# clinfo/kGCN

Hardware: AMD Instinct MI355X
Metric: graphs/sec GraphConv fwd+bwd, 32-node mol graphs x64 feat (higher is better)
Workload: dtype f32

## Files before the change

include/kgcn_hip.h:

```cpp
#ifndef KGCN_HIP_H_
#define KGCN_HIP_H_

#include <stdint.h>

#ifdef __cplusplus
extern "C" {
#endif

#define KGCN_HIP_ABI_VERSION 2

#define KGCN_PAD_COL 32

#define KGCN_ROW_PAD_COMPACT 0x104
#define KGCN_CSR_UNIT_VALUES 1


typedef struct kgcn_csr_batch {
  int32_t num_graphs;
  int32_t rows;
  int32_t cols;
  int32_t max_nnz_per_graph;
  int32_t row_pad;
  int32_t reserved_;
  int64_t nnz;
// ... 123 lines not shown
int kgcn_dense_fwd_act_f32(const float* x, int64_t m, int32_t din, int64_t x_ld, const float* w, int64_t w_ld,
                           int32_t trans_w, const float* bias, float* y, int32_t dout, int64_t y_ld, int32_t act,
                           void* stream);
int64_t kgcn_dense_fwd_workspace_bytes(int32_t din, int32_t dout);
int kgcn_dense_fwd_ws_f32(const float* x, int64_t m, int32_t din, int64_t x_ld, const float* w, int64_t w_ld,
                          int32_t trans_w, const float* bias, float* y, int32_t dout, int64_t y_ld, int32_t act,
                          void* workspace, int64_t workspace_bytes, void* stream);
#define KGCN_WTABLE_MAX_JOBS 16
typedef struct kgcn_wtable_job {
  const float* w;
  int64_t w_ld;
  int32_t trans_w, k, n;
  int32_t k_w;
  void* table;
  const float* extra_row;
} kgcn_wtable_job;
int kgcn_wtable_split_multi(const kgcn_wtable_job* jobs, int32_t num_jobs, void* stream);
int kgcn_dense_fwd_tab_f32(const float* x, int64_t m, int32_t din, int64_t x_ld, const float* w, int64_t w_ld,
                           int32_t trans_w, const float* bias, float* y, int32_t dout, int64_t y_ld, int32_t act,
                           const void* table, int64_t table_bytes, void* stream);
int kgcn_dense_dx_dact_f32(const float* grad, const float* act_out, int64_t m, int32_t dout, int64_t ld, const float* w,
                           int64_t w_ld, int32_t din, float* dx, int64_t dx_ld, int32_t act, float* dpre,
                           void* workspace, int64_t workspace_bytes, void* stream);
int kgcn_dense_dx_dact_tab_f32(const float* grad, const float* act_out, int64_t m, int32_t dout, int64_t ld, const float* w,
                               int64_t w_ld, int32_t din, float* dx, int64_t dx_ld, int32_t act, float* dpre, const void* table,
                               int64_t table_bytes, void* stream);
int kgcn_dense_dx_dact_gather_supported(int64_t m, int32_t din, int32_t dout);
int kgcn_dense_dx_dact_gather_f32(const float* grad, const float* pooled_grad, int64_t pooled_ld, int32_t n_nodes,
                                  const float* act_out, int64_t m, int32_t dout, int64_t ld, const float* w, int64_t w_ld,
                                  int32_t din, float* dx, int64_t dx_ld, int32_t act, float* dpre, void* table,
                                  int64_t table_bytes, int32_t table_ready, void* stream);
int kgcn_dense_bwd_supported(int64_t m, int32_t din, int32_t dout);
int kgcn_dense_bwd_f32(const float* grad, const float* pooled_grad, int64_t pooled_ld, int32_t n_nodes, const float* act_out,
                       int32_t act, int64_t ld, const float* x, int64_t x_ld, int64_t m, int32_t din, int32_t dout,
                       const float* w, int64_t w_ld, float* dx, int64_t dx_ld, float* dw, float* dbias, void* table,
                       int64_t table_bytes, int32_t table_ready, void* workspace, int64_t workspace_bytes, void* stream);
int kgcn_dense_bwd_dot_f32(const float* grad, const float* act_out, int32_t act, int64_t ld, const float* x, int64_t x_ld, int64_t m,
                           int32_t din, int32_t dout, const float* w, int64_t w_ld, const float* dotx, int64_t dotx_ld, float* dw,
                           float* dbias, float* dot_out, void* table, int64_t table_bytes, int32_t table_ready, void* workspace,
                           int64_t workspace_bytes, void* stream);
int kgcn_dense_dx_dact_dot_supported(int64_t m, int32_t din, int32_t dout);
int64_t kgcn_dense_dx_dact_dot_workspace_bytes(int64_t m, int32_t din);
int kgcn_dense_dx_dact_dot_f32(const float* grad, const float* act_out, int64_t m, int32_t dout, int64_t ld, const float* w,
                               int64_t w_ld, int32_t din, const float* dotx, int64_t dotx_ld, int32_t act, float* dpre,
                               void* table, int64_t table_bytes, int32_t table_ready, float* dot_out, void* workspace,
                               int64_t workspace_bytes, void* stream);
int kgcn_act_fwd_f32(const float* x, int64_t n, int32_t act, float* y, void* stream);
int kgcn_act_bwd_f32(const float* act_out, const float* grad, int64_t n, int32_t act, float* dpre, void* stream);

int64_t kgcn_graph_bn_workspace_bytes(int32_t d);
int kgcn_graph_bn_stats_f32(const float* x, int64_t graphs, int32_t n_nodes, int32_t d, const int32_t* enabled,
                            float* mean, float* var, void* workspace, int64_t workspace_bytes, void* stream);
int kgcn_graph_bn_apply_f32(const float* x, int64_t graphs, int32_t n_nodes, int32_t d, const int32_t* enabled,
                            const float* mean, const float* var, const float* gamma, const float* beta, float eps,
                            float* y, void* stream);
int kgcn_graph_bn_bwd_f32(const float* x, const float* grad, int64_t graphs, int32_t n_nodes, int32_t d,
                          const int32_t* enabled, const float* mean, const float* var, const float* gamma, float eps,
                          int32_t training, float* dx, float* dgamma, float* dbeta, void* workspace,
                          int64_t workspace_bytes, void* stream);

int kgcn_graph_bn_apply_act_f32(const float* x, int64_t graphs, int32_t n_nodes, int32_t d, const int32_t* enabled,
                                const float* mean, const float* var, const float* gamma, const float* beta, float eps,
                                int32_t act, float* y, void* stream);
int kgcn_graph_bn_bwd_dact_f32(const float* x, const float* grad, const float* act_out, int32_t act, int64_t graphs,
                               int32_t n_nodes, int32_t d, const int32_t* enabled, const float* mean, const float* var,
                               const float* gamma, float eps, int32_t training, float* dx, float* dgamma, float* dbeta,
                               void* workspace, int64_t workspace_bytes, void* stream);

int64_t kgcn_coo_pack_workspace_bytes(int64_t nnz, int32_t num_graphs, int32_t rows, int32_t cols);
int kgcn_coo_pack_f32(const int32_t* graph, const int32_t* row, const int32_t* col, const float* val, int64_t nnz,
                      int32_t num_graphs, int32_t rows, int32_t cols, int32_t transposed, int32_t* rowptr_out,
                      void* cv_out, int32_t* perm_out, int32_t* stats_out, void* workspace, int64_t workspace_bytes,
                      void* stream);
int64_t kgcn_csr_pad4_workspace_bytes(int32_t num_graphs, int32_t rows);
int kgcn_csr_pad4(const kgcn_csr_batch* a, int32_t* rowptr4_out, void* cv4_out, int64_t cv4_capacity,
                  int32_t* slots_out, int32_t* graph_ptr_out, int32_t* stats_out, void* workspace,
                  int64_t workspace_bytes, void* stream);
int64_t kgcn_compact_values_offset(int64_t nnz);
int64_t kgcn_compact_cv_words(int64_t nnz, int32_t with_values);
int kgcn_csr_compact4(const kgcn_csr_batch* a4, void* cv_out, int with_values, void* slots_out, int32_t* stats_out,
                      void* stream);
int kgcn_graphconv_fused_reads_compact(int32_t backward, int32_t num_graphs, int32_t n_nodes, int32_t din, int32_t dout,
                                       int32_t max_nnz_per_graph, int32_t with_dx);

int64_t kgcn_ragged_workspace_bytes(int32_t num_sel);
int kgcn_ragged_plan(const kgcn_csr_batch* src, const int32_t* sizes, const int32_t* sel, int32_t num_sel,
                     int32_t* graph_ptr, int32_t* entry_ptr, void* workspace, int64_t workspace_bytes, void* stream);
int kgcn_ragged_compact_csr(const kgcn_csr_batch* src, const int32_t* sel, int32_t num_sel, const int32_t* graph_ptr,
                            const int32_t* entry_ptr, int32_t capacity_rows, int32_t* dst_rowptr, int32_t* dst_cv,
                            int64_t dst_cv_capacity, int32_t* status, void* stream);
int kgcn_ragged_compact_csr_pair(const kgcn_csr_batch* src, const kgcn_csr_batch* src_t, const int32_t* sel, int32_t num_sel,
                                 const int32_t* graph_ptr, const int32_t* entry_ptr, int32_t capacity_rows, int32_t* dst_rowptr,
                                 int32_t* dst_cv, int64_t dst_cv_capacity, int32_t* dst_t_rowptr, int32_t* dst_t_cv,
                                 int64_t dst_t_cv_capacity, int32_t* status, void* stream);
#define KGCN_RAGGED_BLOCK_ROWS 32
int32_t kgcn_ragged_block_rows(void);
int32_t kgcn_ragged_num_blocks(int32_t capacity_rows);
int kgcn_ragged_blocks(const int32_t* graph_ptr, int32_t num_sel, int32_t capacity_rows, int32_t* block_ptr, void* stream);
int kgcn_ragged_compact_rows_f32(const float* src, const int32_t* sel, int32_t num_sel, int32_t n_nodes, int32_t d,
                                 const int32_t* graph_ptr, int32_t capacity_rows, float* dst, void* stream);
int kgcn_ragged_compact_rows_aug_f32(const float* src, const int32_t* sel, int32_t num_sel, int32_t n_nodes, int32_t d,
                                     const int32_t* graph_ptr, int32_t capacity_rows, float* dst, int32_t dst_ld, void* stream);
int kgcn_ragged_expand_rows_f32(const float* src, int32_t num_graphs, int32_t n_nodes, int32_t d,
                                const int32_t* graph_ptr, int32_t fill_row, float* dst, void* stream);
int kgcn_ragged_gather_fwd_f32(const float* x, const int32_t* graph_ptr, int64_t batch, int32_t n_nodes, int32_t d,
                               int32_t pad_row, float* out, void* stream);
int64_t kgcn_ragged_gather_bwd_workspace_bytes(int32_t d);
int kgcn_ragged_gather_bwd_f32(const float* dout_grad, const int32_t* graph_ptr, int64_t batch, int32_t n_nodes, int32_t d,
                               int32_t pad_row, int32_t capacity_rows, float* dx, void* workspace, int64_t workspace_bytes,
                               void* stream);

int64_t kgcn_loss_workspace_bytes(int64_t batch);
int kgcn_masked_sigmoid_ce_f32(const float* logits, const float* labels, const float* mask, const float* mask_label,
                               int64_t batch, int32_t tasks, int32_t weighted, float pos_weight,
                               const float* pos_weight_per_task, float* cost, float* dlogits, float* sums, void* workspace,
                               int64_t workspace_bytes, void* stream);
int kgcn_masked_softmax_ce_f32(const float* logits, const float* labels, const float* mask, int64_t batch, int32_t classes,
                               float* cost, float* dlogits, float* sums, void* workspace, int64_t workspace_bytes,
                               void* stream);
int kgcn_sparse_softmax_ce_f32(const float* logits, const int64_t* label_idx, const float* mask, int64_t batch,
                               int32_t classes, float* cost, float* dlogits, float* sums, void* workspace,
                               int64_t workspace_bytes, void* stream);
int kgcn_loss_grad_f32(const float* dlogits, const float* g_opt, const float* g_sum, int64_t batch, int64_t n, float* out,
                       void* stream);
int kgcn_adam_tf_f32(float* params, const float* grads, float* m, float* v, int64_t n, float lr, float beta1, float beta2,
                     float eps, int64_t* step_counter, void* stream);
#define KGCN_ADAM_MAX_SEGMENTS 32
typedef struct kgcn_adam_segment {
  const float* grad;
  int64_t offset, numel;
} kgcn_adam_segment;
int kgcn_adam_tf_multi_f32(float* params, float* m, float* v, int64_t n, const kgcn_adam_segment* segments, int32_t num_segments,
                           float lr, float beta1, float beta2, float eps, int64_t* step_counter, void* stream);

int kgcn_augment_ones_f32(const float* x, int64_t m, int32_t din, int64_t x_ld, float* out, int64_t out_ld, void* stream);
int kgcn_augment_ones_bwd_f32(const float* dout_grad, int64_t m, int32_t din, int64_t g_ld, float* dx, int64_t dx_ld,
                              void* stream);

#define KGCN_STACK_MAX_LAYERS 8
typedef struct kgcn_stack_layer {
  int32_t kind, act, din, dout;
  const float* w;
  const float* b;
  const float* mean;
  const float* var;
  float eps;
  int32_t route;
} kgcn_stack_layer;
int kgcn_gcn_stack_supported(int32_t n_nodes, int32_t max_nnz_per_graph, const kgcn_stack_layer* layers, int32_t num_layers);
int64_t kgcn_gcn_stack_param_floats(const kgcn_stack_layer* layers, int32_t num_layers);
int kgcn_gcn_stack_fwd_f32(const kgcn_csr_batch* a, const float* x, const int32_t* enabled, const kgcn_stack_layer* layers,
                           int32_t num_layers, float* const* layer_out, float* pooled, void* stream);
int64_t kgcn_gcn_stack_bwd_workspace_bytes(int32_t num_graphs, const kgcn_stack_layer* layers, int32_t num_layers);
int kgcn_gcn_stack_bwd_f32(const kgcn_csr_batch* at, const float* x, const int32_t* enabled, const kgcn_stack_layer* layers,
                           int32_t num_layers, float* const* layer_out, const float* dlast, int32_t gather, float* dx,
                           float* dparams, void* workspace, int64_t workspace_bytes, void* stream);

int kgcn_reduce_defer(int32_t on);
int kgcn_reduce_pending(void);
int kgcn_reduce_flush(void* stream);

int kgcn_dense_mfma_products(int32_t kind, int64_t m, int32_t din, int32_t dout);

enum {
  KGCN_SPMM_NONE = 0,
  KGCN_SPMM_TILE = 1,
// ... 227 lines not shown
```

kgcn_amd/csrc/fused.hip:

```cpp
#include <type_traits>

#include "kgcn_common.h"
#include "kgcn_probe.h"

namespace kgcn {

constexpr int FN = 32;
constexpr int FD = 64;
constexpr int ALD = 68;
constexpr int BLD = 65;
constexpr int MAX_WPB = 8;


KP_BUFFER(g_probe, kgcn_probe_set)

__device__ __forceinline__ void wave_sync() {
  __builtin_amdgcn_wave_barrier();
  asm volatile("" ::: "memory");
  __builtin_amdgcn_wave_barrier();
}

typedef int i32x4 __attribute__((ext_vector_type(4)));

__device__ __forceinline__ f32x4 ldv4(const float* p) { return *reinterpret_cast<const f32x4*>(p); }
// ... 276 lines not shown
      x1 = ldv4(reinterpret_cast<const float*>(sb + (cw[0] >> 16)));
      x2 = ldv4(reinterpret_cast<const float*>(sb + (cw[1] & 0xffffu)));
      x3 = ldv4(reinterpret_cast<const float*>(sb + (cw[1] >> 16)));
    }
  }
  template <int I>
  __device__ __forceinline__ float val() const {
    if constexpr (LAY == LAY_PAD4) return __int_as_float(I == 0 ? q0.y : I == 1 ? q0.w : I == 2 ? q1.y : q1.w);
    else return v[I];
  }
  __device__ __forceinline__ void fma() {
    if constexpr (LAY == LAY_UNIT) {
      a = x0;
      add4(a, x1); add4(a, x2); add4(a, x3);
    } else {
      const float v0 = val<0>();
      a[0] = v0 * x0[0]; a[1] = v0 * x0[1]; a[2] = v0 * x0[2]; a[3] = v0 * x0[3];
      fma4(a, val<1>(), x1);
      fma4(a, val<2>(), x2);
      fma4(a, val<3>(), x3);
    }
  }
};
template <int LAY>
__device__ __forceinline__ f32x4 gather4(const int2* ecv, const float* ev, const float* srcl, int k) {
  Grp4<LAY> q;
  q.ecv(ecv, ev, k);
  q.tile(srcl);
  f32x4 a0 = {0.f, 0.f, 0.f, 0.f};
  if constexpr (LAY == LAY_UNIT) {
    add4(a0, q.x0); add4(a0, q.x1); add4(a0, q.x2); add4(a0, q.x3);
  } else {
    fma4(a0, q.template val<0>(), q.x0); fma4(a0, q.template val<1>(), q.x1);
    fma4(a0, q.template val<2>(), q.x2); fma4(a0, q.template val<3>(), q.x3);
  }
  return a0;
}
template <int LAY>
__device__ __forceinline__ void grp_tail(f32x4& a, int s, int len, const int2* ecv, const float* ev, const float* srcl) {
  if (__builtin_amdgcn_ballot_w64(len > 4)) {
    for (int k = 4; __builtin_amdgcn_ballot_w64(k < len); k += 4)
      if (k < len) add4(a, gather4<LAY>(ecv, ev, srcl, s + k));
  }
}

template <typename Emit>
__device__ __forceinline__ void aggregate_rows(const int2* ecv, const int* tab, const float* tile,
                                               int N, int dcols, int lane, Emit&& emit) {
  const int sub = lane >> 4, cl = lane & 15;
  const float* srcl = tile + cl * 4;
  const bool col_ok = cl * 4 < dcols;
  for (int j0 = 0; j0 < N; j0 += 4) {
    const int j = j0 + sub;
    const bool ok = (j < N) && col_ok;
    int s_, len, row;
    unpack_slot(tab[ok ? j : 0], s_, len, row);
    if (!ok) len = 0;
    f32x4 acc = {0.f, 0.f, 0.f, 0.f};
    for (int k = 0; __builtin_amdgcn_ballot_w64(k < len); k += 4)
      if (k < len) add4(acc, gather4<LAY_PAD4>(ecv, nullptr, srcl, s_ + k));
    if (ok) emit(row, cl, acc);
  }
}

template <int LAY, typename Emit>
__device__ __forceinline__ void aggregate_rows_full(const int2* ecv, const float* ev, const int* tab, const float* tile,
                                                    int lane, Emit&& emit) {
  const int sub = lane >> 4, cl = lane & 15;
  const float* srcl = tile + cl * 4;
#pragma unroll
  for (int p8 = 0; p8 < 8; ++p8) {
    int s, len, row;
    unpack_slot(tab[4 * p8 + sub], s, len, row);
    Grp4<LAY> q;
    q.ecv(ecv, ev, s);
    q.tile(srcl);
    q.fma();
    grp_tail<LAY>(q.a, s, len, ecv, ev, srcl);
    emit(row, cl, q.a);
    __builtin_amdgcn_sched_barrier(0);
  }
}

constexpr int A_FWD = FN * ALD;
constexpr int A_BWD = FN * BLD;

template <bool FULL>
__device__ __forceinline__ void load_w_frags(float (&wr0)[32], float (&wr1)[32],
                                             const float* __restrict__ w, int din, int dout, int li,
                                             int hi) {
#pragma unroll
  for (int s = 0; s < 32; ++s) {
    const int k = hi * 32 + s;
    if constexpr (FULL) {
      wr0[s] = w[k * FD + li];
      wr1[s] = w[k * FD + 32 + li];
    } else {
      wr0[s] = (k < din && li < dout) ? w[(long)k * dout + li] : 0.f;
      wr1[s] = (k < din && 32 + li < dout) ? w[(long)k * dout + 32 + li] : 0.f;
    }
  }
}

__device__ __forceinline__ void store_c_tiles(float* tile, const f32x16& c0, const f32x16& c1, int li,
                                              int hi) {
#pragma unroll
  for (int r = 0; r < 16; ++r) {
    const int row = (r & 3) + 8 * (r >> 2) + 4 * hi;
    tile[row * FD + li] = c0[r];
    tile[row * FD + 32 + li] = c1[r];
  }
}

template <int MODE>
__global__ __launch_bounds__(512, 2) void graphconv_fwd_kernel(
    const int* __restrict__ slots, const int* __restrict__ gptr, const int2* __restrict__ cv,
    const float* __restrict__ x, const float* __restrict__ w, const float* __restrict__ bias,
    float* __restrict__ out, int T, int N, int din, int dout, int max_nnz, int pack) {
  constexpr bool VEC = MODE == 2;
  extern __shared__ __attribute__((aligned(16))) unsigned char smem[];
  const int tid = threadIdx.x;
  const int wave = tid >> 6, lane = tid & 63;
  const int li = lane & 31, hi = lane >> 5;
  const int wpb = blockDim.x >> 6;
  WaveSlice ws = carve(smem, wave, max_nnz * pack, A_FWD, 1);

  const int stride = gridDim.x * wpb * pack;
  int t = __builtin_amdgcn_readfirstlane((blockIdx.x * wpb + wave) * pack);
  if (t >= T) return;

  for (int i = lane; i < A_FWD; i += 64) ws.a[i] = 0.f;
  for (int i = lane; i < FD; i += 64) ws.b[FN * FD + i] = 0.f;

  float wr0[32], wr1[32];
  load_w_frags<false>(wr0, wr1, w, din, dout, li, hi);
  const float b0 = (bias && li < dout) ? bias[li] : 0.f;
  const float b1 = (bias && 32 + li < dout) ? bias[32 + li] : 0.f;

  auto graphs_at = [&](int tt) { return T - tt < pack ? T - tt : pack; };
  int P = graphs_at(t);

  TileRegs fx;
  CsrRegs fc;
  MetaRegs m_cur, m_nxt;
  issue_meta_p(m_cur, slots, gptr, t, P, N, lane);
  int base = meta_base(m_cur), cnt = meta_cnt_p(m_cur, P);
  issue_tile_g<MODE>(fx, x + (long)t * N * din, P * N * din, lane);
  issue_cv(fc, cv, base, cnt, lane);
  int tn = t + stride;
  int Pn = graphs_at(tn < T ? tn : t);
  issue_meta_p(m_nxt, slots, gptr, tn < T ? tn : t, Pn, N, lane);
  wave_sync();

  for (;;) {
    const int rows = P * N;
    land_tile_g<MODE>(fx, ws.a, ALD, rows * din, din, lane);
    land_csr_p(fc, ws.ecv, ws.rp, cv, m_cur, base, cnt, N, P, lane);
    wave_sync();

    const bool has_next = tn < T;
    const int tp = has_next ? tn : t;
    const int base_n = meta_base(m_nxt), cnt_n = meta_cnt_p(m_nxt, Pn);
    issue_tile_g<MODE>(fx, x + (long)tp * N * din, Pn * N * din, lane);
    issue_cv(fc, cv, base_n, cnt_n, lane);
    m_cur = m_nxt;
    const int P_next = Pn;
    {
      const int tnn = tn + stride;
      const int tq = tnn < T ? tnn : tp;
      Pn = graphs_at(tq);
      issue_meta_p(m_nxt, slots, gptr, tq, Pn, N, lane);
    }

    f32x16 acc0, acc1;
#pragma unroll
    for (int r = 0; r < 16; ++r) { acc0[r] = b0; acc1[r] = b1; }
    {
      f32x4 a4[8];
#pragma unroll
      for (int q = 0; q < 8; ++q) a4[q] = ldv4(ws.a + li * ALD + hi * 32 + q * 4);
#pragma unroll
      for (int s = 0; s < 32; ++s) {
        const float a = a4[s >> 2][s & 3];
        acc0 = __builtin_amdgcn_mfma_f32_32x32x2f32(a, wr0[s], acc0, 0, 0, 0);
        acc1 = __builtin_amdgcn_mfma_f32_32x32x2f32(a, wr1[s], acc1, 0, 0, 0);
      }
    }
    store_c_tiles(ws.b, acc0, acc1, li, hi);
    wave_sync();

    float* ot = out + (long)t * N * dout;
    aggregate_rows(ws.ecv, ws.rp, ws.b, rows, dout, lane, [&](int r, int cl, f32x4 acc) {
      if constexpr (VEC) {
        stv4(ot + (long)r * dout + cl * 4, acc);
      } else {
#pragma unroll
        for (int j = 0; j < 4; ++j)
          if (cl * 4 + j < dout) ot[(long)r * dout + cl * 4 + j] = acc[j];
      }
    });
    wave_sync();

    if (!has_next) break;
    t = tn;
    tn += stride;
    P = P_next;
    base = base_n;
    cnt = cnt_n;
  }
}

constexpr size_t FWD_FULL_SHARED = 2 * 4 * 64 * 16;

template <int LAY>
__global__ __launch_bounds__(512, 2) void graphconv_fwd_full_kernel(
    const int* __restrict__ slots, const int* __restrict__ gptr, const int2* __restrict__ cv,
    const float* __restrict__ cvals, const float* __restrict__ x, const float* __restrict__ w,
    const float* __restrict__ bias, float* __restrict__ out, int T, int max_nnz) {
  extern __shared__ __attribute__((aligned(16))) unsigned char smem[];
  constexpr int N = FN, D = FD;
  const int tid = threadIdx.x;
  const int wave = tid >> 6, lane = tid & 63;
  const int li = lane & 31, hi = lane >> 5;
  const int wpb = blockDim.x >> 6;
  u32x4* w3 = reinterpret_cast<u32x4*>(smem);
  WaveSlice ws = carve(smem + FWD_FULL_SHARED, wave, max_nnz, A_FWD, 1);
  const float* ev = reinterpret_cast<const float*>(reinterpret_cast<unsigned char*>(ws.ecv) + cvals_off(max_nnz));
  const unsigned* cw = reinterpret_cast<const unsigned*>(cv);
  using CsrIn = std::conditional_t<LAY == LAY_PAD4, CsrRegs, CsrRegsC>;
  auto issue_csr = [&](CsrIn& f, int b_, int c_) __attribute__((always_inline)) {
    if constexpr (LAY == LAY_PAD4) issue_cv(f, cv, b_, c_, lane);
    else issue_cv_c<LAY>(f, cw, cvals, b_, c_, lane);
  };

  u32x4 WF[2][4][2];
  static_for<8>([&](auto c) __attribute__((always_inline)) {
    constexpr int nt = decltype(c)::value >> 2, ks = decltype(c)::value & 3;
    float v[8];
#pragma unroll
    for (int j = 0; j < 8; ++j) v[j] = w[(16 * ks + 8 * hi + j) * D + 32 * nt + li];
    Frag3 f;
    split8(v, f);
    WF[nt][ks][0] = f.p1; WF[nt][ks][1] = f.p2;
    if (wave == 0) w3[(nt * 4 + ks) * 64 + lane] = f.p3;
  });
  __syncthreads();

  const int nwaves = gridDim.x * wpb;
  int t = __builtin_amdgcn_readfirstlane(blockIdx.x * wpb + wave);
  if (t >= T) return;
#ifdef KGCN_ABL_HOT
  const int t_first = t;
  auto hot = [&](int tt) { return t_first + (((tt - t_first) / nwaves) & 1) * nwaves < T ? t_first + (((tt - t_first) / nwaves) & 1) * nwaves : t_first; };
#else
  auto hot = [&](int tt) { return tt; };
#endif

  for (int i = lane; i < D; i += 64) ws.b[FN * FD + i] = 0.f;
  const float b0 = bias ? bias[li] : 0.f;
  const float b1 = bias ? bias[32 + li] : 0.f;

  TileRegs fx;
  CsrIn fc;
  MetaRegs m_cur, m_nxt;
  issue_meta_l<LAY>(m_cur, slots, gptr, hot(t), N, lane);
  int base = meta_base(m_cur), cnt = meta_cnt(m_cur);
  issue_tile<true, true>(fx, x + (long)hot(t) * N * D, 512, lane);
  issue_csr(fc, base, cnt);
  int tn = t + nwaves;
  issue_meta_l<LAY>(m_nxt, slots, gptr, hot(tn < T ? tn : t), N, lane);
  wave_sync();

  int t_prev = t;
  bool has_next = true;
  KP_DECL(8)
  auto aggregate_prev = [&]() __attribute__((always_inline)) {
    float* ot = out + (long)hot(t_prev) * N * D;
    aggregate_rows_full<LAY>(ws.ecv, ev, ws.rp, ws.b, lane, [&](int r, int c4, f32x4 v) {
      stv4_stream(ot + r * D + c4 * 4, v);
    });
  };
  auto step = [&](auto agg_tag) __attribute__((always_inline)) {
    constexpr bool AGG = decltype(agg_tag)::value;
    KP_STAMP(0)
    land_tile<true>(fx, ws.a, ALD, 512, 16, lane);
    has_next = tn < T;
    const int tp = has_next ? tn : t;
    static_assert(FD * FD >= FN * FD, "W holds at least one tile's floats");
    issue_tile<true, true>(fx, has_next ? x + (long)hot(tn) * N * D : w, 512, lane);
    wave_sync();
    KP_STAMP(1)

    if constexpr (AGG) aggregate_prev();
    wave_sync();
    KP_STAMP(2)

    if constexpr (LAY == LAY_PAD4) land_csr(fc, ws.ecv, ws.rp, cv, m_cur.slot, base, cnt, N, lane);
    else land_csr_c<LAY>(fc, ws.ecv, ws.rp, cw, cvals, max_nnz, compact_slot_word(m_cur.slot), base, cnt, N, lane);
    const int base_n = meta_base(m_nxt), cnt_n = meta_cnt(m_nxt);
    issue_csr(fc, base_n, cnt_n);
    asm volatile("v_mov_b32 %0, %2\n\tv_mov_b32 %1, %3"
                 : "=&v"(m_cur.slot), "=&v"(m_cur.gp) : "v"(m_nxt.slot), "v"(m_nxt.gp));
    {
      const int tnn = tn + nwaves;
      issue_meta_l<LAY>(m_nxt, slots, gptr, hot(tnn < T ? tnn : tp), N, lane);
    }

    f32x16 acc0, acc1;
#pragma unroll
    for (int r = 0; r < 16; ++r) { acc0[r] = b0; acc1[r] = b1; }
    static_for<4>([&](auto ksc) __attribute__((always_inline)) {
      constexpr int ks = decltype(ksc)::value;
      const float* src = ws.a + li * ALD + 16 * ks + 8 * hi;
      const f32x4 lo = ldv4(src), hi4 = ldv4(src + 4);
      const float v[8] = {lo[0], lo[1], lo[2], lo[3], hi4[0], hi4[1], hi4[2], hi4[3]};
      Frag3 fa;
      split8(v, fa);
      const u32x4 w30 = w3[ks * 64 + lane], w31 = w3[(4 + ks) * 64 + lane];
      acc0 = mfma_bf16(fa.p3, WF[0][ks][0], acc0);
      acc1 = mfma_bf16(fa.p3, WF[1][ks][0], acc1);
      acc0 = mfma_bf16(fa.p2, WF[0][ks][1], acc0);
      acc1 = mfma_bf16(fa.p2, WF[1][ks][1], acc1);
      acc0 = mfma_bf16(fa.p1, w30, acc0);
      acc1 = mfma_bf16(fa.p1, w31, acc1);
      acc0 = mfma_bf16(fa.p2, WF[0][ks][0], acc0);
      acc1 = mfma_bf16(fa.p2, WF[1][ks][0], acc1);
      acc0 = mfma_bf16(fa.p1, WF[0][ks][1], acc0);
      acc1 = mfma_bf16(fa.p1, WF[1][ks][1], acc1);
      acc0 = mfma_bf16(fa.p1, WF[0][ks][0], acc0);
      acc1 = mfma_bf16(fa.p1, WF[1][ks][0], acc1);
      __builtin_amdgcn_sched_barrier(0);
    });
    KP_STAMP(3)
    store_c_tiles(ws.b, acc0, acc1, li, hi);
    wave_sync();
    KP_STAMP(4)

    t_prev = t;
    t = tn;
    tn += nwaves;
    base = base_n;
    cnt = cnt_n;
  };

  step(std::false_type{});
  while (has_next) step(std::true_type{});
  aggregate_prev();
  KP_FLUSH(g_probe, blockIdx.x * wpb + wave, 8)
}

template <int MODE>
__global__ __launch_bounds__(512, 2) void graphconv_bwd_kernel(
    const int* __restrict__ slots_t, const int* __restrict__ gptr_t, const int2* __restrict__ cv_t,
    const float* __restrict__ x, const float* __restrict__ w, const float* __restrict__ g,
    float* __restrict__ dx, float* __restrict__ part_dw, float* __restrict__ part_db, int T, int N,
    int din, int dout, int max_nnz, int pack) {
  constexpr bool VEC = MODE == 2;
  extern __shared__ __attribute__((aligned(16))) unsigned char smem[];
  const int tid = threadIdx.x;
  const int wave = tid >> 6, lane = tid & 63;
  const int li = lane & 31, hi = lane >> 5;
  const int wpb = blockDim.x >> 6;
  float* Wt = reinterpret_cast<float*>(smem);
  WaveSlice ws = carve(smem + FD * FD * 4, wave, max_nnz * pack, A_BWD, 1);

  for (int i = tid; i < FD * FD; i += blockDim.x) {
    const int k = i >> 6, j = i & 63;
    Wt[i] = (j < din && k < dout) ? w[(long)j * dout + k] : 0.f;
  }
  for (int i = lane; i < A_BWD; i += 64) ws.a[i] = 0.f;
  for (int i = lane; i < (FN + 1) * FD; i += 64) ws.b[i] = 0.f;
  __syncthreads();

  f32x16 dw00, dw01, dw10, dw11;
#pragma unroll
  for (int r = 0; r < 16; ++r) { dw00[r] = 0.f; dw01[r] = 0.f; dw10[r] = 0.f; dw11[r] = 0.f; }
  f32x4 dbacc = {0.f, 0.f, 0.f, 0.f};

  const int din4 = din >> 2;
  const int stride = gridDim.x * wpb * pack;
  int t = __builtin_amdgcn_readfirstlane((blockIdx.x * wpb + wave) * pack);

  if (t < T) {
    auto graphs_at = [&](int tt) { return T - tt < pack ? T - tt : pack; };
    int P = graphs_at(t);
    TileRegs fg, fx;
    CsrRegs fc;
    MetaRegs m_cur, m_nxt;
    issue_meta_p(m_cur, slots_t, gptr_t, t, P, N, lane);
    int base = meta_base(m_cur), cnt = meta_cnt_p(m_cur, P);
    issue_tile_g<MODE>(fg, g + (long)t * N * dout, P * N * dout, lane);
    issue_cv(fc, cv_t, base, cnt, lane);
    issue_tile_g<MODE>(fx, x + (long)t * N * din, P * N * din, lane);
    int tn = t + stride;
    int Pn = graphs_at(tn < T ? tn : t);
    issue_meta_p(m_nxt, slots_t, gptr_t, tn < T ? tn : t, Pn, N, lane);

    KP_DECL(8)
    for (;;) {
      KP_STAMP(0)
      const int rows = P * N;
      const int nxe = rows * din, nge = rows * dout, nx4 = rows * din4;
      land_tile_g<MODE>(fg, ws.b, FD, nge, dout, lane);
      land_csr_p(fc, ws.ecv, ws.rp, cv_t, m_cur, base, cnt, N, P, lane);
      if (P < pack) {
        for (int i = rows * BLD + lane; i < pack * N * BLD; i += 64) ws.a[i] = 0.f;
      }
      wave_sync();

      KP_STAMP(1)
      aggregate_rows(ws.ecv, ws.rp, ws.b, rows, dout, lane, [&](int r, int cl, f32x4 acc) {
        float* d = ws.a + r * BLD + cl * 4;
        d[0] = acc[0]; d[1] = acc[1]; d[2] = acc[2]; d[3] = acc[3];
        dbacc += acc;
      });
// ... 927 lines not shown
          constexpr int pa = ks == 0 ? PA0[pr] : PA1[pr], pb = ks == 0 ? PB0[pr] : PB1[pr];
          const u32x4 av = XF[ks][tile >> 1][pa];
          const u32x4 bv = ks == 0 ? BF0[tile & 1][pb] : BF1[tile & 1][pb];
          if constexpr (tile == 0) dw00 = mfma_bf16(av, bv, dw00);
          else if constexpr (tile == 1) dw01 = mfma_bf16(av, bv, dw01);
          else if constexpr (tile == 2) dw10 = mfma_bf16(av, bv, dw10);
          else dw11 = mfma_bf16(av, bv, dw11);
          if constexpr (ks == 0 && (m == 12 || m == 13 || m == 20 || m == 21 || m == 22 || m == 23)) {
            constexpr int pc = m < 14 ? 2 : m < 22 ? 1 : 0;
            read_bf(BF1, std::integral_constant<int, 1>{}, std::integral_constant<int, (m & 1)>{},
                    std::integral_constant<int, pc>{}, cur_off);
          }
        });
      });
    };

    __syncthreads();
    {
      const float* xb = x + (long)gidx(0) * N * D + xlane;
      static_for<16>([&](auto qc) __attribute__((always_inline)) { load_x(xb, qc); });
    }
    split_and_reload(1);
    if (lane == 0) { *agg_flag = 0; *spare_word = 0; }
    bp_barrier();

    int cur = 0;
    KP_STAMP(0)
    for (int i = 0; i < cnt_max - 1; ++i) {
      if (i < cnt_max - 2 || whole) {
        aggregate(MB{}, ecv0 + (cur ^ 1) * ecv_stride, tab0 + (cur ^ 1) * (FN + 4), cur ? 0u : (unsigned)DFWP_BYTES);
        wave_sync();
        if (lane == 0) *agg_flag = i + 1;
      }
      KP_STAMP(3)
      dw_of(cur);
      KP_STAMP(1)
      split_and_reload(i + 2);
      KP_STAMP(2)
      bp_barrier();
      KP_STAMP(4)
      cur ^= 1;
    }
    if (whole) dw_of(cur);
    KP_STAMP(5)
  }
  KP_FLUSH(g_probe, blockIdx.x * 8 + wave, 8)

  __syncthreads();
  float* park = reinterpret_cast<float*>(sl);
  if (role == 1) {
#pragma unroll
    for (int r = 0; r < 16; ++r) {
      const int row = (r & 3) + 8 * (r >> 2) + 4 * hi;
      park[(2 * row) * FD + li] = dw00[r];
      park[(2 * row) * FD + 32 + li] = dw01[r];
      park[(2 * row + 1) * FD + li] = dw10[r];
      park[(2 * row + 1) * FD + 32 + li] = dw11[r];
    }
  }
#pragma unroll
  for (int j = 0; j < 4; ++j) {
    float v = dbacc[j];
    v += __shfl_xor(v, 16, 64);
    v += __shfl_xor(v, 32, 64);
    dbacc[j] = v;
  }
  if (lane < 16) stv4(park + FD * FD + role * FD + lane * 4, dbacc);
  __syncthreads();
  const size_t slice_f = 2 * DFWP_BYTES / 4;
  const float* slice0 = reinterpret_cast<const float*>(smem);
  float* pw = part_dw + (long)blockIdx.x * D * D;
  for (int i = tid; i < D * D; i += blockDim.x) {
    float s = 0.f;
    for (int wv = 0; wv < BP_PAIRS; ++wv) s += slice0[wv * slice_f + i];
    pw[i] = s;
  }
  if (tid < D) {
    float s = 0.f;
    for (int wv = 0; wv < BP_PAIRS; ++wv) s += slice0[wv * slice_f + D * D + tid] + slice0[wv * slice_f + D * D + D + tid];
    part_db[(long)blockIdx.x * D + tid] = s;
  }
}

static int fused_wpb(size_t per_wave, size_t shared_bytes) {
  long fit = ((long)kLdsBytes - (long)shared_bytes) / (long)per_wave;
  if (fit > MAX_WPB) fit = MAX_WPB;
  return fit < 1 ? 0 : (int)fit;
}

static int fused_grid(int T, int wpb) {
  int blocks = (T + wpb - 1) / wpb;
  if (blocks > kNumCU) blocks = kNumCU;
  return blocks < 1 ? 1 : blocks;
}

static bool is_full(int n, int din, int dout) { return n == FN && din == FD && dout == FD; }

static int pack_factor(int n, int max_nnz, size_t a_floats_shared) {
  int p = FN / n;
  if (p > MAX_PACK) p = MAX_PACK;
  while (p > 1) {
    const size_t per = slice_bytes(max_nnz * p, a_floats_shared == 0 ? A_FWD : A_BWD, 1);
    long fit = ((long)kLdsBytes - (long)a_floats_shared) / (long)per;
    if (fit >= 4 && (long)max_nnz * p < 65536) break;
    --p;
  }
  return p < 1 ? 1 : p;
}

static size_t fwd_slice(int, int, int, int max_nnz) { return slice_bytes(max_nnz, A_FWD, 1); }
static size_t fwd_shared(int n, int din, int dout) { return is_full(n, din, dout) ? FWD_FULL_SHARED : 0; }
static size_t bwd_slice(int max_nnz) { return slice_bytes(max_nnz, A_BWD, 1); }

static bool fused_shape_ok(int n, int din, int dout, int max_nnz) {
  if (n <= 0 || n > FN) return false;
  if (din <= 0 || din > FD) return false;
  if (dout <= 0 || dout > FD) return false;
  if (max_nnz < 0 || (max_nnz & 3)) return false;
  return fused_wpb(fwd_slice(n, din, dout, max_nnz), fwd_shared(n, din, dout)) >= 4 &&
         fused_wpb(bwd_slice(max_nnz), FD * FD * 4) >= 4;
}

template <typename F>
static void with_const3(int v, F&& f) {
  if (v == 2) f(std::integral_constant<int, 2>{});
  else if (v == 1) f(std::integral_constant<int, 1>{});
  else f(std::integral_constant<int, 0>{});
}
static_assert(LAY_PAD4 == 0 && LAY_UNIT == 1 && LAY_VALS == 2, "with_const3 covers the three layouts");

static bool is_compact(const kgcn_csr_batch* a) { return a->row_pad == KGCN_ROW_PAD_COMPACT; }

static int check_padded(const kgcn_csr_batch* a, const char* who) {
  if (!a) return validate_csr(a, who, true);
  kgcn_csr_batch v = *a;
  if (is_compact(a)) v.row_pad = 4;
  if (int rc = validate_csr(&v, who, true)) return rc;
  if (a->row_pad != 4 && !is_compact(a))
    return fail("%s: the fused kernels read the row-padded layout (row_pad = 4 or the compact %d), got row_pad=%d", who,
                KGCN_ROW_PAD_COMPACT, a->row_pad);
  if (is_compact(a) && (a->reserved_ & ~KGCN_CSR_UNIT_VALUES))
    return fail("%s: unknown flags 0x%x in a compact batch", who, (unsigned)a->reserved_);
  if (a->num_graphs > 0 && (!a->slots || !a->graph_ptr))
    return fail("%s: row-padded batch without slots / graph_ptr", who);
  if (a->rows != a->cols) return fail("%s: adjacency must be square", who);
  return 0;
}

static int lay_of(const kgcn_csr_batch* a) {
  return !is_compact(a) ? LAY_PAD4 : (a->reserved_ & KGCN_CSR_UNIT_VALUES) ? LAY_UNIT : LAY_VALS;
}
static const float* compact_values(const kgcn_csr_batch* a) {
  return lay_of(a) == LAY_VALS ? reinterpret_cast<const float*>(a->cv + kgcn_compact_values_offset(a->nnz)) : nullptr;
}

static bool bwd_full_route(int n, int din, int dout, int max_nnz, bool with_dx) {
  return with_dx && is_full(n, din, dout) && bwd_planes_lds_bytes(max_nnz) <= (size_t)kLdsBytes && max_nnz < 4096;
}
static bool bwd_pairs_route(int T, int n, int din, int dout, int max_nnz, bool with_dx) {
  return bwd_full_route(n, din, dout, max_nnz, with_dx) &&
         T >= 2 * BP_PAIRS * fused_grid(T, BWD_FULL_WPB);
}

}

using namespace kgcn;

extern "C" int64_t kgcn_compact_values_offset(int64_t nnz) { return ((nnz / 4) + 3) & ~(int64_t)3; }

extern "C" int64_t kgcn_compact_cv_words(int64_t nnz, int32_t with_values) {
  return with_values ? kgcn_compact_values_offset(nnz) + nnz : nnz / 4;
}

extern "C" int kgcn_graphconv_fused_reads_compact(int32_t backward, int32_t num_graphs, int32_t n_nodes, int32_t din,
                                                  int32_t dout, int32_t max_nnz_per_graph, int32_t with_dx) {
  if (num_graphs <= 0 || !fused_shape_ok(n_nodes, din, dout, max_nnz_per_graph)) return 0;
  if (!backward) return is_full(n_nodes, din, dout) ? 1 : 0;
  return bwd_pairs_route(num_graphs, n_nodes, din, dout, max_nnz_per_graph, with_dx != 0) ? 1 : 0;
}

extern "C" int kgcn_graphconv_fused_supported(int32_t n_nodes, int32_t din, int32_t dout,
                                              int32_t max_nnz_per_graph) {
  return fused_shape_ok(n_nodes, din, dout, (max_nnz_per_graph + 3) & ~3) ? 1 : 0;
}

extern "C" int kgcn_graphconv_fwd_f32(const kgcn_csr_batch* a, const float* x, const float* w,
                                      const float* bias, int32_t din, int32_t dout, float* out,
                                      void* stream) {
  if (int rc = check_padded(a, "kgcn_graphconv_fwd_f32")) return rc;
  if (!fused_shape_ok(a->rows, din, dout, a->max_nnz_per_graph))
    return fail("kgcn_graphconv_fwd_f32: shape N=%d din=%d dout=%d max_nnz=%d not supported by the "
                "fused kernel (use kgcn_dense_fwd_f32 + kgcn_bconv_f32)",
                a->rows, din, dout, a->max_nnz_per_graph);
  if (a->num_graphs == 0) return 0;
  if (!x || !w || !out) return fail("kgcn_graphconv_fwd_f32: NULL operand");
  const bool vec = !(din & 3) && !(dout & 3);
  if ((vec && (!aligned16(x) || !aligned16(out))) || !aligned16(a->cv))
    return fail("kgcn_graphconv_fwd_f32: x/out/cv not 16-byte aligned");
  const int mode = vec ? 2 : (((a->rows * din) & 3) == 0 && ((a->rows * dout) & 3) == 0 && aligned16(x)) ? 1 : 0;
  const bool full_shape = is_full(a->rows, din, dout);
  if (is_compact(a) && !full_shape)
    return fail("kgcn_graphconv_fwd_f32: the compact adjacency layout is read by the FULL-shape kernel only (N=%d din=%d "
                "dout=%d): pass the row-padded batch", a->rows, din, dout);
  const int pack = full_shape ? 1 : pack_factor(a->rows, a->max_nnz_per_graph, 0);
  const size_t per = fwd_slice(a->rows, din, dout, a->max_nnz_per_graph * pack);
  const size_t shared = fwd_shared(a->rows, din, dout);
  const int wpb = fused_wpb(per, shared);
  const size_t lds = shared + (size_t)wpb * per;
  const int tiles = (a->num_graphs + pack - 1) / pack;
  const dim3 grid(fused_grid(tiles, wpb)), block(64 * wpb);
  const int2* cv = reinterpret_cast<const int2*>(a->cv);
  const int lay = lay_of(a);
  const float* cvals = compact_values(a);
  int rc = 0;
  if (full_shape)
    with_const3(lay, [&](auto L) {
      constexpr auto kernel = graphconv_fwd_full_kernel<decltype(L)::value>;
      if ((rc = allow_full_lds<kernel>(lds, "graphconv_fwd_full_kernel"))) return;
      hipLaunchKernelGGL(kernel, grid, block, lds, as_stream(stream), a->slots, a->graph_ptr, cv, cvals, x, w, bias, out,
                         a->num_graphs, a->max_nnz_per_graph);
    });
  else
    with_const3(mode, [&](auto M) {
      constexpr auto kernel = graphconv_fwd_kernel<decltype(M)::value>;
      if ((rc = allow_full_lds<kernel>(lds, "graphconv_fwd_kernel"))) return;
      hipLaunchKernelGGL(kernel, grid, block, lds, as_stream(stream), a->slots, a->graph_ptr, cv, x, w, bias, out, a->num_graphs,
                         a->rows, din, dout, a->max_nnz_per_graph, pack);
    });
  if (rc) return rc;
  return check_launch("graphconv_fwd_kernel");
}

extern "C" int64_t kgcn_graphconv_bwd_workspace_bytes(int32_t num_graphs, int32_t din,
                                                      int32_t dout) {
  if (num_graphs <= 0 || din <= 0 || dout <= 0) return 0;
  return (int64_t)kNumCU * ((int64_t)din * dout + dout) * 4;
}

extern "C" int kgcn_graphconv_bwd_f32(const kgcn_csr_batch* at, const float* x, const float* w,
                                      const float* dout_grad, int32_t din, int32_t dout, float* dx,
                                      float* dw, float* dbias, void* workspace,
                                      int64_t workspace_bytes, void* stream) {
  if (int rc = check_padded(at, "kgcn_graphconv_bwd_f32")) return rc;
  if (!fused_shape_ok(at->rows, din, dout, at->max_nnz_per_graph))
    return fail("kgcn_graphconv_bwd_f32: shape N=%d din=%d dout=%d max_nnz=%d not supported by the "
                "fused kernel", at->rows, din, dout, at->max_nnz_per_graph);
  if (!dw || !dbias) return fail("kgcn_graphconv_bwd_f32: dw/dbias is NULL");
  hipStream_t s = as_stream(stream);
  if (at->num_graphs == 0) {
    (void)hipMemsetAsync(dw, 0, (size_t)din * dout * 4, s);
    (void)hipMemsetAsync(dbias, 0, (size_t)dout * 4, s);
    return 0;
  }
  if (!x || !w || !dout_grad) return fail("kgcn_graphconv_bwd_f32: NULL operand");
  const bool vec = !(din & 3) && !(dout & 3);
  if ((vec && (!aligned16(x) || !aligned16(dout_grad) || (dx && !aligned16(dx)))) || !aligned16(at->cv))
    return fail("kgcn_graphconv_bwd_f32: tensors not 16-byte aligned");
  const int mode = vec ? 2 : (((at->rows * din) & 3) == 0 && ((at->rows * dout) & 3) == 0 && aligned16(x) &&
                              aligned16(dout_grad) && (!dx || aligned16(dx))) ? 1 : 0;
  const size_t full_lds = bwd_planes_lds_bytes(at->max_nnz_per_graph);
  const bool full = bwd_full_route(at->rows, din, dout, at->max_nnz_per_graph, dx != nullptr);
  const int pack = (full || is_full(at->rows, din, dout)) ? 1 : pack_factor(at->rows, at->max_nnz_per_graph, FD * FD * 4);
  const size_t per = full ? full_lds / BWD_FULL_WPB : bwd_slice(at->max_nnz_per_graph * pack);
  const int wpb = full ? BWD_FULL_WPB : fused_wpb(per, FD * FD * 4);
  const int blocks = fused_grid((at->num_graphs + pack - 1) / pack, wpb);
  const bool pairs = bwd_pairs_route(at->num_graphs, at->rows, din, dout, at->max_nnz_per_graph, dx != nullptr);
  if (is_compact(at) && !pairs)
    return fail("kgcn_graphconv_bwd_f32: the compact adjacency layout is read by the pairs kernel only (T=%d N=%d din=%d "
                "dout=%d, dx %s): pass the row-padded batch", at->num_graphs, at->rows, din, dout, dx ? "wanted" : "NULL");
  const int64_t need = (int64_t)blocks * ((int64_t)din * dout + dout) * 4;
  if (!workspace || workspace_bytes < need)
    return fail("kgcn_graphconv_bwd_f32: workspace %lld < %lld bytes", (long long)workspace_bytes,
                (long long)need);
  float* part_dw = static_cast<float*>(workspace);
  float* part_db = part_dw + (long)blocks * din * dout;
  const size_t lds = full ? full_lds : FD * FD * 4 + (size_t)wpb * per;
  const int2* cv = reinterpret_cast<const int2*>(at->cv);
  const int lay = lay_of(at);
  const float* cvals = compact_values(at);
  int rc = 0;
  if (pairs)
    with_const3(lay, [&](auto L) {
      auto go = [&](auto streams) {
        constexpr auto kernel = graphconv_bwd_pairs_kernel<decltype(L)::value, decltype(streams)::value>;
        if ((rc = allow_full_lds<kernel>(lds, "graphconv_bwd_pairs_kernel"))) return;
        hipLaunchKernelGGL(kernel, dim3(blocks), dim3(512), lds, s, at->slots, at->graph_ptr, cv, cvals, x, w, dout_grad, dx,
                           part_dw, part_db, at->num_graphs, at->max_nnz_per_graph);
      };
      if (bwd_streams(at->num_graphs)) go(std::true_type{}); else go(std::false_type{});
    });
  else if (full) {
    if ((rc = allow_full_lds<graphconv_bwd_planes_kernel>(lds, "graphconv_bwd_planes_kernel"))) return rc;
    hipLaunchKernelGGL(graphconv_bwd_planes_kernel, dim3(blocks), dim3(64 * wpb), lds, s, at->slots,
                       at->graph_ptr, cv, x, w, dout_grad, dx, part_dw, part_db, at->num_graphs,
                       at->max_nnz_per_graph);
  } else
    with_const3(mode, [&](auto M) {
      constexpr auto kernel = graphconv_bwd_kernel<decltype(M)::value>;
      if ((rc = allow_full_lds<kernel>(lds, "graphconv_bwd_kernel"))) return;
      hipLaunchKernelGGL(kernel, dim3(blocks), dim3(64 * wpb), lds, s, at->slots, at->graph_ptr, cv, x, w, dout_grad, dx, part_dw,
                         part_db, at->num_graphs, at->rows, din, dout, at->max_nnz_per_graph, pack);
// ... 6 lines not shown
```

Measured before the change: 130.0 million.

## Add producer/consumer wave-pair forward GraphConv kernel for large batches

Adds a new full-shape forward kernel in which waves are split into pairs. One wave of each pair loads tiles and CSR data and runs the MFMA dense contraction into a double-buffered LDS tile. The partner wave aggregates rows from the previous tile and streams them to output. It also adds a two-rows-at-a-time aggregation helper and a look-ahead LDS load in the contraction. The new kernel is used only when the batch is large (at least 16384 graphs by default) and its LDS need fits. In exchange it brings extra barrier synchronisation and more LDS per block, and smaller batches keep the old per-wave kernel.

```diff
diff --git a/include/kgcn_hip.h b/include/kgcn_hip.h
--- a/include/kgcn_hip.h
+++ b/include/kgcn_hip.h
@@ -229,6 +229,7 @@
                       void* stream);
 int kgcn_graphconv_fused_reads_compact(int32_t backward, int32_t num_graphs, int32_t n_nodes, int32_t din, int32_t dout,
                                        int32_t max_nnz_per_graph, int32_t with_dx);
+int kgcn_graphconv_fwd_pairs_route(int32_t num_graphs, int32_t n_nodes, int32_t din, int32_t dout, int32_t max_nnz_per_graph);
 
 int64_t kgcn_ragged_workspace_bytes(int32_t num_sel);
 int kgcn_ragged_plan(const kgcn_csr_batch* src, const int32_t* sizes, const int32_t* sel, int32_t num_sel,
diff --git a/kgcn_amd/csrc/fused.hip b/kgcn_amd/csrc/fused.hip
--- a/kgcn_amd/csrc/fused.hip
+++ b/kgcn_amd/csrc/fused.hip
@@ -382,6 +382,31 @@
   }
 }
 
+template <int LAY, typename Emit>
+__device__ __forceinline__ void aggregate_rows_full2(const int2* ecv, const float* ev, const int* tab, const float* tile,
+                                                     int lane, Emit&& emit) {
+  const int sub = lane >> 4, cl = lane & 15;
+  const float* srcl = tile + cl * 4;
+#pragma unroll
+  for (int p4 = 0; p4 < 4; ++p4) {
+    int sa, lena, rowa, sb, lenb, rowb;
+    unpack_slot(tab[8 * p4 + sub], sa, lena, rowa);
+    unpack_slot(tab[8 * p4 + 4 + sub], sb, lenb, rowb);
+    Grp4<LAY> qa, qb;
+    qa.ecv(ecv, ev, sa);
+    qb.ecv(ecv, ev, sb);
+    qa.tile(srcl);
+    qb.tile(srcl);
+    qa.fma();
+    qb.fma();
+    grp_tail<LAY>(qa.a, sa, lena, ecv, ev, srcl);
+    grp_tail<LAY>(qb.a, sb, lenb, ecv, ev, srcl);
+    emit(rowa, cl, qa.a);
+    emit(rowb, cl, qb.a);
+    __builtin_amdgcn_sched_barrier(0);
+  }
+}
+
 constexpr int A_FWD = FN * ALD;
 constexpr int A_BWD = FN * BLD;
 
@@ -410,6 +435,53 @@
     tile[row * FD + li] = c0[r];
     tile[row * FD + 32 + li] = c1[r];
   }
+}
+
+__device__ __forceinline__ void fwd_w_frags(u32x4 (&WF)[2][4][2], u32x4* w3, bool table, const float* __restrict__ w, int lane) {
+  const int li = lane & 31, hi = lane >> 5;
+  static_for<8>([&](auto c) __attribute__((always_inline)) {
+    constexpr int nt = decltype(c)::value >> 2, ks = decltype(c)::value & 3;
+    float v[8];
+#pragma unroll
+    for (int j = 0; j < 8; ++j) v[j] = w[(16 * ks + 8 * hi + j) * FD + 32 * nt + li];
+    Frag3 f;
+    split8(v, f);
+    WF[nt][ks][0] = f.p1; WF[nt][ks][1] = f.p2;
+    if (table) w3[(nt * 4 + ks) * 64 + lane] = f.p3;
+  });
+}
+template <bool AHEAD = false>
+__device__ __forceinline__ void fwd_contract(f32x16& acc0, f32x16& acc1, const float* a, const u32x4 (&WF)[2][4][2],
+                                             const u32x4* w3, float b0, float b1, int lane) {
+  const int li = lane & 31, hi = lane >> 5;
+#pragma unroll
+  for (int r = 0; r < 16; ++r) { acc0[r] = b0; acc1[r] = b1; }
+  const float* src0 = a + li * ALD + 8 * hi;
+  f32x4 lo, hi4;
+  if constexpr (AHEAD) { lo = ldv4(src0); hi4 = ldv4(src0 + 4); }
+  static_for<4>([&](auto ksc) __attribute__((always_inline)) {
+    constexpr int ks = decltype(ksc)::value;
+    const float* src = src0 + 16 * ks;
+    if constexpr (!AHEAD) { lo = ldv4(src); hi4 = ldv4(src + 4); }
+    const float v[8] = {lo[0], lo[1], lo[2], lo[3], hi4[0], hi4[1], hi4[2], hi4[3]};
+    if constexpr (AHEAD && ks < 3) { lo = ldv4(src + 16); hi4 = ldv4(src + 20); }
+    Frag3 fa;
+    split8(v, fa);
+    const u32x4 w30 = w3[ks * 64 + lane], w31 = w3[(4 + ks) * 64 + lane];
+    acc0 = mfma_bf16(fa.p3, WF[0][ks][0], acc0);
+    acc1 = mfma_bf16(fa.p3, WF[1][ks][0], acc1);
+    acc0 = mfma_bf16(fa.p2, WF[0][ks][1], acc0);
+    acc1 = mfma_bf16(fa.p2, WF[1][ks][1], acc1);
+    acc0 = mfma_bf16(fa.p1, w30, acc0);
+    acc1 = mfma_bf16(fa.p1, w31, acc1);
+    acc0 = mfma_bf16(fa.p2, WF[0][ks][0], acc0);
+    acc1 = mfma_bf16(fa.p2, WF[1][ks][0], acc1);
+    acc0 = mfma_bf16(fa.p1, WF[0][ks][1], acc0);
+    acc1 = mfma_bf16(fa.p1, WF[1][ks][1], acc1);
+    acc0 = mfma_bf16(fa.p1, WF[0][ks][0], acc0);
+    acc1 = mfma_bf16(fa.p1, WF[1][ks][0], acc1);
+    __builtin_amdgcn_sched_barrier(0);
+  });
 }
 
 template <int MODE>
@@ -513,7 +585,7 @@
 constexpr size_t FWD_FULL_SHARED = 2 * 4 * 64 * 16;
 
 template <int LAY>
-__global__ __launch_bounds__(512, 2) void graphconv_fwd_full_kernel(
+__global__ __launch_bounds__(512, 2) void graphconv_fwd_wave_kernel(
     const int* __restrict__ slots, const int* __restrict__ gptr, const int2* __restrict__ cv,
     const float* __restrict__ cvals, const float* __restrict__ x, const float* __restrict__ w,
     const float* __restrict__ bias, float* __restrict__ out, int T, int max_nnz) {
@@ -534,16 +606,7 @@
   };
 
   u32x4 WF[2][4][2];
-  static_for<8>([&](auto c) __attribute__((always_inline)) {
-    constexpr int nt = decltype(c)::value >> 2, ks = decltype(c)::value & 3;
-    float v[8];
-#pragma unroll
-    for (int j = 0; j < 8; ++j) v[j] = w[(16 * ks + 8 * hi + j) * D + 32 * nt + li];
-    Frag3 f;
-    split8(v, f);
-    WF[nt][ks][0] = f.p1; WF[nt][ks][1] = f.p2;
-    if (wave == 0) w3[(nt * 4 + ks) * 64 + lane] = f.p3;
-  });
+  fwd_w_frags(WF, w3, wave == 0, w, lane);
   __syncthreads();
 
   const int nwaves = gridDim.x * wpb;
@@ -607,30 +670,7 @@
     }
 
     f32x16 acc0, acc1;
-#pragma unroll
-    for (int r = 0; r < 16; ++r) { acc0[r] = b0; acc1[r] = b1; }
-    static_for<4>([&](auto ksc) __attribute__((always_inline)) {
-      constexpr int ks = decltype(ksc)::value;
-      const float* src = ws.a + li * ALD + 16 * ks + 8 * hi;
-      const f32x4 lo = ldv4(src), hi4 = ldv4(src + 4);
-      const float v[8] = {lo[0], lo[1], lo[2], lo[3], hi4[0], hi4[1], hi4[2], hi4[3]};
-      Frag3 fa;
-      split8(v, fa);
-      const u32x4 w30 = w3[ks * 64 + lane], w31 = w3[(4 + ks) * 64 + lane];
-      acc0 = mfma_bf16(fa.p3, WF[0][ks][0], acc0);
-      acc1 = mfma_bf16(fa.p3, WF[1][ks][0], acc1);
-      acc0 = mfma_bf16(fa.p2, WF[0][ks][1], acc0);
-      acc1 = mfma_bf16(fa.p2, WF[1][ks][1], acc1);
-      acc0 = mfma_bf16(fa.p1, w30, acc0);
-      acc1 = mfma_bf16(fa.p1, w31, acc1);
-      acc0 = mfma_bf16(fa.p2, WF[0][ks][0], acc0);
-      acc1 = mfma_bf16(fa.p2, WF[1][ks][0], acc1);
-      acc0 = mfma_bf16(fa.p1, WF[0][ks][1], acc0);
-      acc1 = mfma_bf16(fa.p1, WF[1][ks][1], acc1);
-      acc0 = mfma_bf16(fa.p1, WF[0][ks][0], acc0);
-      acc1 = mfma_bf16(fa.p1, WF[1][ks][0], acc1);
-      __builtin_amdgcn_sched_barrier(0);
-    });
+    fwd_contract(acc0, acc1, ws.a, WF, w3, b0, b1, lane);
     KP_STAMP(3)
     store_c_tiles(ws.b, acc0, acc1, li, hi);
     wave_sync();
@@ -1724,6 +1764,119 @@
   }
 }
 
+constexpr int FP_PAIRS = 4;
+constexpr size_t FP_GT_FLOATS = (size_t)(FN + 1) * FD;
+__host__ __device__ inline size_t fwd_pairs_pair_bytes(int max_nnz) {
+  return (size_t)A_FWD * 4 + 2 * FP_GT_FLOATS * 4 + 2 * (ecv_bytes(max_nnz) + RP_BYTES);
+}
+static_assert((A_FWD * 4) % 16 == 0 && (FP_GT_FLOATS * 4) % 16 == 0 && RP_BYTES % 16 == 0, "16-byte aligned LDS regions");
+static size_t fwd_pairs_lds_bytes(int max_nnz) { return FWD_FULL_SHARED + FP_PAIRS * fwd_pairs_pair_bytes(max_nnz); }
+
+template <int LAY>
+__global__ __launch_bounds__(512, 2) void graphconv_fwd_full_kernel(
+    const int* __restrict__ slots, const int* __restrict__ gptr, const int2* __restrict__ cv,
+    const float* __restrict__ cvals, const float* __restrict__ x, const float* __restrict__ w,
+    const float* __restrict__ bias, float* __restrict__ out, int T, int max_nnz) {
+  extern __shared__ __attribute__((aligned(16))) unsigned char smem[];
+  constexpr int N = FN, D = FD;
+  const int tid = threadIdx.x;
+  const int wave = __builtin_amdgcn_readfirstlane(tid >> 6), lane = tid & 63;
+  const int pair = wave & 3, role = wave >> 2;
+  const int li = lane & 31, hi = lane >> 5;
+  u32x4* w3 = reinterpret_cast<u32x4*>(smem);
+  float* at = reinterpret_cast<float*>(smem + FWD_FULL_SHARED + (size_t)pair * fwd_pairs_pair_bytes(max_nnz));
+  float* gt0 = at + A_FWD;
+  int2* ecv0 = reinterpret_cast<int2*>(gt0 + 2 * FP_GT_FLOATS);
+  const size_t ecv_stride = ecv_bytes(max_nnz) / 8;
+  int* tab0 = reinterpret_cast<int*>(reinterpret_cast<unsigned char*>(ecv0) + 2 * ecv_bytes(max_nnz));
+
+  const int npairs = gridDim.x * FP_PAIRS;
+  const int t0 = blockIdx.x * FP_PAIRS + pair;
+  const int cnt_max = (T - 1) / npairs + 1;
+  const int cntw = (T - 1 - t0) / npairs + 1;
+  const int tl = t0 + (cntw - 1) * npairs;
+  const bool whole = cntw == cnt_max;
+  auto gidx = [&](int k) { return graph_at(t0, npairs, tl, k); };
+
+  if (role == 0) {
+    u32x4 WF[2][4][2];
+    fwd_w_frags(WF, w3, pair == 0, w, lane);
+    if (lane < D) { gt0[FN * FD + lane] = 0.f; gt0[FP_GT_FLOATS + FN * FD + lane] = 0.f; }
+    __syncthreads();
+    const float b0 = bias ? bias[li] : 0.f;
+    const float b1 = bias ? bias[32 + li] : 0.f;
+    const unsigned* cw = reinterpret_cast<const unsigned*>(cv);
+    using CsrIn = std::conditional_t<LAY == LAY_PAD4, CsrRegs, CsrRegsC>;
+    auto issue_csr = [&](CsrIn& f, int b_, int c_) __attribute__((always_inline)) {
+      if constexpr (LAY == LAY_PAD4) issue_cv(f, cv, b_, c_, lane);
+      else issue_cv_c<LAY>(f, cw, cvals, b_, c_, lane);
+    };
+    TileRegs fx;
+    CsrIn fc;
+    MetaRegs m_cur, m_nxt;
+    issue_meta_l<LAY>(m_cur, slots, gptr, gidx(0), N, lane);
+    int base = meta_base(m_cur), cnt = meta_cnt(m_cur);
+    issue_tile<true, true>(fx, x + (long)gidx(0) * N * D, 512, lane);
+    issue_csr(fc, base, cnt);
+    issue_meta_l<LAY>(m_nxt, slots, gptr, gidx(1), N, lane);
+    wave_sync();
+    auto land_csr_l = [&](int cur) __attribute__((always_inline)) {
+      int2* ecv_c = ecv0 + cur * ecv_stride;
+      int* tab_c = tab0 + cur * (FN + 4);
+      if constexpr (LAY == LAY_PAD4) land_csr(fc, ecv_c, tab_c, cv, m_cur.slot, base, cnt, N, lane);
+      else land_csr_c<LAY>(fc, ecv_c, tab_c, cw, cvals, max_nnz, compact_slot_word(m_cur.slot), base, cnt, N, lane);
+    };
+    auto multiply = [&](int cur) __attribute__((always_inline)) {
+      f32x16 acc0, acc1;
+      fwd_contract<true>(acc0, acc1, at, WF, w3, b0, b1, lane);
+      store_c_tiles(gt0 + cur * FP_GT_FLOATS, acc0, acc1, li, hi);
+    };
+    int cur = 0;
+    for (int i = 0; i < cnt_max - 1; ++i) {
+      land_tile<true>(fx, at, ALD, 512, 16, lane);
+      static_assert(FD * FD >= FN * FD, "W holds at least one tile's floats");
+      issue_tile<true, true>(fx, i + 1 < cntw ? x + (long)gidx(i + 1) * N * D : w, 512, lane);
+      wave_sync();
+      land_csr_l(cur);
+      const int base_n = meta_base(m_nxt), cnt_n = meta_cnt(m_nxt);
+      issue_csr(fc, base_n, cnt_n);
+      asm volatile("v_mov_b32 %0, %2\n\tv_mov_b32 %1, %3"
+                   : "=&v"(m_cur.slot), "=&v"(m_cur.gp) : "v"(m_nxt.slot), "v"(m_nxt.gp));
+      issue_meta_l<LAY>(m_nxt, slots, gptr, gidx(i + 2), N, lane);
+      multiply(cur);
+      base = base_n;
+      cnt = cnt_n;
+      bp_barrier();
+      cur ^= 1;
+    }
+    if (whole) {
+      land_tile<true>(fx, at, ALD, 512, 16, lane);
+      wave_sync();
+      land_csr_l(cur);
+      multiply(cur);
+    }
+    bp_barrier();
+  } else {
+    __syncthreads();
+    auto aggregate = [&](int k, int cur) __attribute__((always_inline)) {
+      float* ot = out + (long)gidx(k) * N * D;
+      const int2* ecv_c = ecv0 + cur * ecv_stride;
+      const float* ev = reinterpret_cast<const float*>(reinterpret_cast<const unsigned char*>(ecv_c) + cvals_off(max_nnz));
+      aggregate_rows_full2<LAY>(ecv_c, ev, tab0 + cur * (FN + 4), gt0 + cur * FP_GT_FLOATS, lane, [&](int r, int c4, f32x4 v) {
+        stv4_stream(ot + r * D + c4 * 4, v);
+      });
+    };
+    bp_barrier();
+    int cur = 0;
+    for (int i = 1; i < cnt_max; ++i) {
+      aggregate(i - 1, cur);
+      bp_barrier();
+      cur ^= 1;
+    }
+    if (whole) aggregate(cnt_max - 1, cur);
+  }
+}
+
 static int fused_wpb(size_t per_wave, size_t shared_bytes) {
   long fit = ((long)kLdsBytes - (long)shared_bytes) / (long)per_wave;
   if (fit > MAX_WPB) fit = MAX_WPB;
@@ -1804,6 +1957,14 @@
          T >= 2 * BP_PAIRS * fused_grid(T, BWD_FULL_WPB);
 }
 
+#ifndef KGCN_FWD_PAIRS_MIN_GRAPHS
+#define KGCN_FWD_PAIRS_MIN_GRAPHS 16384
+#endif
+static bool fwd_pairs_route(int T, int n, int din, int dout, int max_nnz) {
+  return is_full(n, din, dout) && fwd_pairs_lds_bytes(max_nnz) <= (size_t)kLdsBytes && T >= KGCN_FWD_PAIRS_MIN_GRAPHS &&
+         T >= 2 * FP_PAIRS * fused_grid(T, FP_PAIRS);
+}
+
 }
 
 using namespace kgcn;
@@ -1819,6 +1980,12 @@
   if (num_graphs <= 0 || !fused_shape_ok(n_nodes, din, dout, max_nnz_per_graph)) return 0;
   if (!backward) return is_full(n_nodes, din, dout) ? 1 : 0;
   return bwd_pairs_route(num_graphs, n_nodes, din, dout, max_nnz_per_graph, with_dx != 0) ? 1 : 0;
+}
+
+extern "C" int kgcn_graphconv_fwd_pairs_route(int32_t num_graphs, int32_t n_nodes, int32_t din, int32_t dout,
+                                              int32_t max_nnz_per_graph) {
+  if (num_graphs <= 0 || !fused_shape_ok(n_nodes, din, dout, max_nnz_per_graph)) return 0;
+  return fwd_pairs_route(num_graphs, n_nodes, din, dout, max_nnz_per_graph) ? 1 : 0;
 }
 
 extern "C" int kgcn_graphconv_fused_supported(int32_t n_nodes, int32_t din, int32_t dout,
@@ -1855,10 +2022,18 @@
   const int lay = lay_of(a);
   const float* cvals = compact_values(a);
   int rc = 0;
-  if (full_shape)
+  if (fwd_pairs_route(a->num_graphs, a->rows, din, dout, a->max_nnz_per_graph))
     with_const3(lay, [&](auto L) {
       constexpr auto kernel = graphconv_fwd_full_kernel<decltype(L)::value>;
-      if ((rc = allow_full_lds<kernel>(lds, "graphconv_fwd_full_kernel"))) return;
+      const size_t pairs_lds = fwd_pairs_lds_bytes(a->max_nnz_per_graph);
+      if ((rc = allow_full_lds<kernel>(pairs_lds, "graphconv_fwd_full_kernel"))) return;
+      hipLaunchKernelGGL(kernel, dim3(fused_grid(a->num_graphs, FP_PAIRS)), dim3(128 * FP_PAIRS), pairs_lds, as_stream(stream),
+                         a->slots, a->graph_ptr, cv, cvals, x, w, bias, out, a->num_graphs, a->max_nnz_per_graph);
+    });
+  else if (full_shape)
+    with_const3(lay, [&](auto L) {
+      constexpr auto kernel = graphconv_fwd_wave_kernel<decltype(L)::value>;
+      if ((rc = allow_full_lds<kernel>(lds, "graphconv_fwd_wave_kernel"))) return;
       hipLaunchKernelGGL(kernel, grid, block, lds, as_stream(stream), a->slots, a->graph_ptr, cv, cvals, x, w, bias, out,
                          a->num_graphs, a->max_nnz_per_graph);
     });
```

Result: faster. 132.8 million, median of 6 (+2.1%).
